# lambdaclass/simpleworks

Hardware: AMD Instinct MI355X
Metric: Marlin prove() constraints/sec at 2^20 R1CS; G1 MSM points/sec (higher is better)
Workload: dtype u32 limbs (384-bit Montgomery Fq for G1, 256-bit Fr); 1 GPU; marlin_prove: synthetic R1CS, 2^20 constraints = variables = non-zeros per matrix (|H| = |K| = 2^20), SRS + proving key device resident; per_gpu_units=1048576, multi_gpu=replicas (one proof per rank)

## Files before the change

### simpleworks_amd/_lib.py

```python
import ctypes
import json
import os

import numpy as np

_HERE = os.path.dirname(os.path.abspath(__file__))
LIB_PATH = os.environ.get("SWM_LIB_PATH") or os.path.join(_HERE, "libswmarlin.so")

_u64p = ctypes.POINTER(ctypes.c_uint64)
_u32p = ctypes.POINTER(ctypes.c_uint32)
_vp = ctypes.c_void_p
_sz = ctypes.c_size_t
_int = ctypes.c_int

ABI = {
    "swm_version": (_int, []),
    "swm_strerror": (ctypes.c_char_p, [_int]),
    "swm_init": (_int, [_int, ctypes.POINTER(_vp)]),
    "swm_destroy": (None, [_vp]),
    "swm_last_error": (ctypes.c_char_p, [_vp]),
    "swm_set_stream": (_int, [_vp, _vp]),
    "swm_set_msm_sharding": (_int, [_vp, ctypes.c_uint, ctypes.c_uint, _vp, _vp]),
    "swm_rccl_unique_id": (_int, [ctypes.c_void_p]),
    "swm_rccl_init": (_int, [_vp, ctypes.c_void_p, ctypes.c_uint, ctypes.c_uint]),
# ... 427 lines not shown
    def selftest_poly_eval(self, p_mont, z_mont):
        p = np.ascontiguousarray(p_mont, dtype=np.uint64).reshape(-1, 4)
        out = np.zeros(4, dtype=np.uint64)
        self._poly(2, p, p.shape[0], 0, z_mont, None, out)
        return out

    def selftest_poly_eval_many(self, buf_mont, pieces, z_mont):
        buf = np.ascontiguousarray(buf_mont, dtype=np.uint64).reshape(-1, 4)
        pc = np.asarray(pieces, dtype=np.uint64).reshape(-1, 2)
        out = np.zeros((pc.shape[0], 4), dtype=np.uint64)
        self._poly(3, buf, buf.shape[0], 0, z_mont, pc, out)
        return out

    def selftest_ntt_from(self, src_mont, log_n, inverse=False, coset=False):
        src = np.ascontiguousarray(src_mont, dtype=np.uint64).reshape(-1, 4).copy()
        out = np.zeros((1 << log_n, 4), dtype=np.uint64)
        self._poly(4 + int(bool(inverse)) + 2 * int(bool(coset)), src, src.shape[0], log_n, None, None, out)
        return out, src

    def selftest_ntt_cosets(self, coeffs_mont, log_n, ks):
        src = np.ascontiguousarray(coeffs_mont, dtype=np.uint64).reshape(-1, 4).copy()
        kk = np.ascontiguousarray(ks, dtype=np.uint64).reshape(-1)
        out = np.zeros((kk.size << log_n, 4), dtype=np.uint64)
        self._check(self.lib.swm_selftest_poly(self.h, 9, src.ctypes.data, src.shape[0], log_n, _p64(np.zeros(4, np.uint64)),
                                               _p64(kk), kk.size, out.ctypes.data), "swm_selftest_poly")
        return out.reshape(kk.size, 1 << log_n, 4)

    def selftest_intt_cosets3(self, evals_mont, log_n):
        ev = np.ascontiguousarray(evals_mont, dtype=np.uint64).reshape(-1, 4).copy()
        out = np.zeros_like(ev)
        self._poly(10, ev, ev.shape[0], log_n, None, None, out)
        return out

    def selftest_scan(self, words):
        w = np.ascontiguousarray(words, dtype=np.uint32).reshape(-1)
        out = np.zeros(w.size + 1, dtype=np.uint32)
        self._poly(8, w, w.size, 0, None, None, out)
        return out[:-1], int(out[-1])

    def selftest_sample_fr(self, rng, need):
        out = np.zeros((max(need, 1), 4), dtype=np.uint64)
        self._check(self.lib.swm_selftest_sample_fr(self.h, rng.h, need, _p64(out)), "swm_selftest_sample_fr")
        return out[:need]

    def selftest_mul_throughput(self, which, threads, iters):
        ms = ctypes.c_float(0)
        self._check(self.lib.swm_selftest_mul_throughput(self.h, which, threads, iters, ctypes.byref(ms)),
                    "swm_selftest_mul_throughput")
        return ms.value
```

### simpleworks_amd/csrc/devops.cuh

```cuda
#pragma once
#include <chrono>
#include <exception>
#include <functional>
#include <utility>
#include <atomic>
#include "context.h"
#include "ff.cuh"
#include "fill.cuh"
#include "fr29.cuh"
#include "host/chacha.h"
#include "host/marlin_types.h"

namespace swm {

int ntt_run(swm_ctx* ctx, void* d_data, unsigned log_n, int inverse, int coset);
int ntt_run_from(swm_ctx* ctx, void* d_data, unsigned log_n, int inverse, int coset, const void* first_src, size_t src_len);
int ntt_cosets_fwd(swm_ctx* ctx, const void* coeffs, size_t len, unsigned log_n, const unsigned* ks, unsigned ncos, void* out);
int ntt_cosets_inv(swm_ctx* ctx, void* data, unsigned log_n, unsigned ncos);
int ntt_sharded_run(swm_ctx* ctx, void* d_local, unsigned log_n, int inverse, int blocks_in);
struct SpmvPlanHost {
    uint64_t nnz = 0, max_row = 0;
    std::vector<uint32_t> chunks, lrows;
};
struct SpmvPlan {
    uint64_t nnz = 0, max_row = 0;
    const uint32_t* d_chunks = nullptr;
    const uint32_t* d_lrows = nullptr;
    uint32_t n_chunks = 0, n_lrows = 0;
};
void spmv_plan_build(const uint32_t* rowptr, size_t rows, SpmvPlanHost* plan);
int spmv_run(swm_ctx* ctx, const void* d_rowptr, const void* d_col, const void* d_val, const void* d_z, void* d_out,
             size_t rows, const SpmvPlan* plan = nullptr);
int batch_inverse_run(swm_ctx* ctx, void* d, size_t n);

inline void hip_check(swm_ctx* ctx, hipError_t e, const char* what) {
    if (e != hipSuccess) {
        set_err(ctx, SWM_ERR_HIP, "%s: %s", what, hipGetErrorString(e));
        throw MarlinError(e == hipErrorOutOfMemory ? SWM_ERR_OOM : SWM_ERR_HIP, std::string(what) + ": " + hipGetErrorString(e));
    }
}
inline void rc_check(swm_ctx* ctx, int rc) {
    if (rc != SWM_OK) throw MarlinError(rc, ctx->err);
}

template <class T>
struct DBuf {
    swm_ctx* ctx = nullptr;
    T* p = nullptr;
    size_t n = 0, cap = 0;
    DBuf() {}
    DBuf(swm_ctx* c, size_t count) : ctx(c), n(count) {
// ... 829 lines not shown
```

### simpleworks_amd/csrc/marlin.hip

```cpp
#include <stdlib.h>
#include <string.h>
#include <unistd.h>
#include <algorithm>
#include <chrono>
#include <functional>
#include <memory>
#include "devops.cuh"
#include "g1.cuh"
#include "host/ahp.h"

#include "msm.h"
using namespace swm;

#define LAUNCHX(ctx, name, kernel, grid, block, shmem, ...)                         \
    do {                                                                            \
        prof_begin(ctx, name);                                                      \
        hipLaunchKernelGGL(kernel, grid, block, shmem, (ctx)->stream, __VA_ARGS__); \
        prof_end(ctx);                                                              \
        hip_check(ctx, hipGetLastError(), name);                                    \
    } while (0)

#include "host/pk_codec.h"
#include "host/host_handles.h"
struct swm_srs {
// ... 1009 lines not shown
        poly[H] = fp_add(poly[H], rho);
    });
}
void div_vh(swm_ctx* ctx, const Fr* q, size_t part, size_t total, Fr* h, Fr* g) {
    ew(ctx, "div_vh", 3 * part, [=] __device__(size_t j) {
        Fr acc = q[j + part];
        if (j + 2 * part < total) acc = fp_add(acc, q[j + 2 * part]);
        if (j + 3 * part < total) acc = fp_add(acc, q[j + 3 * part]);
        h[j] = acc;
        if (j < part) g[j] = fp_add(q[j], acc);
    });
}
void div_vk(swm_ctx* ctx, const Fr* q, size_t part, size_t total, Fr* h) {
    ew(ctx, "div_vk", 3 * part, [=] __device__(size_t j) {
        Fr acc = fp_zero<Fr>();
        for (uint64_t i = 1; j + i * part < total; i++) acc = fp_add(acc, q[j + i * part]);
        h[j] = acc;
    });
}
#ifndef SWM_OUTER_COSETS
#define SWM_OUTER_COSETS 1
#endif
static constexpr uint64_t OUTER_COSETS_MIN_H = 16;
struct Cosets3 {
    Fr p0, p1, p2;
};
__device__ __forceinline__ Cosets3 cosets3_solve(const Fr& u0, const Fr& u1, const Fr& u2, const Fr& iota, const Fr& half) {
    const Fr p1 = fp_mul(fp_sub(u0, u2), half);
    const Fr e = fp_mul(fp_add(u0, u2), half);
    const Fr d = fp_sub(u1, fp_mul(iota, p1));
    return {fp_mul(fp_add(e, d), half), p1, fp_mul(fp_sub(e, d), half)};
}
static Fr fr_half() { return fp_inv(fp_from_u64<Fr>(2)); }
struct RAlphaNumerators {
    Fr n0, n1, n2, n3;
};
RAlphaNumerators r_alpha_numerators(const Fr& alpha, unsigned logH, uint64_t M) {
    Fr aH = alpha;
    for (unsigned i = 0; i < logH; i++) aH = fp_sqr(aH);
    Fr i4 = HDomain(M).gen;
    for (unsigned i = 0; i < logH; i++) i4 = fp_sqr(i4);
    return {fp_sub(aH, fp_one<Fr>()), fp_sub(aH, i4), fp_sub(aH, fp_sqr(i4)), fp_sub(aH, fp_mul(fp_sqr(i4), i4))};
}
struct IndexOnB {
    const Fr *ar, *ac, *arc, *av;
    const Fr *br, *bc, *brc, *bv;
    const Fr *cr, *cc, *crc, *cv;
};
struct Round3Challenges {
    Fr alpha, beta, ab, eta_a, eta_b, eta_c, vhab;
};
__device__ __forceinline__ Fr round3_a_minus_bf(const IndexOnB& x, const Round3Challenges& c, size_t i, const Fr& f) {
    Fr da = fp_add(fp_sub(fp_sub(c.ab, fp_mul(x.ar[i], c.alpha)), fp_mul(c.beta, x.ac[i])), x.arc[i]);
    Fr db = fp_add(fp_sub(fp_sub(c.ab, fp_mul(x.br[i], c.alpha)), fp_mul(c.beta, x.bc[i])), x.brc[i]);
    Fr dc = fp_add(fp_sub(fp_sub(c.ab, fp_mul(x.cr[i], c.alpha)), fp_mul(c.beta, x.cc[i])), x.crc[i]);
    Fr dbc = fp_mul(db, dc);
    Fr t = fp_add(fp_add(fp_mul(fp_mul(c.eta_a, x.av[i]), dbc), fp_mul(fp_mul(fp_mul(c.eta_b, x.bv[i]), da), dc)),
                  fp_mul(fp_mul(fp_mul(c.eta_c, x.cv[i]), da), db));
    Fr a_val = fp_mul(c.vhab, t);
    Fr b_val = fp_mul(da, dbc);
    return fp_sub(a_val, fp_mul(b_val, f));
}
struct ProveState {
    ChaChaRng& zk;
    PhaseTrace& tr;
    const ProveShape shape;
// ... 353 lines not shown
                q[k] = fp_sub(fp_mul(rh[k], summed), fp_mul(zk, th[k]));
            });
        }
        dv_ntt(ctx, s.t_poly, pk.logH, true);
    }
    s.tr.tick("r2: t polynomial enqueued");
    s.P_t.p = s.t_poly.p;
    s.P_t.n = H;
    pc_commit_begin(ctx, pk, &s.lane, s.P_t.p, s.P_t.n, false, 0, false, &s.j2[0]);
}

void round2_q1_cosets(swm_ctx* ctx, const swm_pk& pk, ProveState& s) {
    const uint64_t H = s.H;
    const Fr eta_a = s.st.eta_a, eta_b = s.st.eta_b, eta_c = s.st.eta_c;
    if (!s.ra_closed_form) {
        DVec ra_poly = dv_ntt_from(ctx, s.r_alpha_evals.p, H, pk.logH, true);
        DVec e12 = on_cosets12(ctx, s, ra_poly.p, H);
        s.e_ra = DVec(ctx, 3 * H);
        hip_check(ctx, hipMemcpyAsync(s.e_ra.p + H, e12.p, 2 * H * sizeof(Fr), hipMemcpyDeviceToDevice, ctx->stream), "copy");
    }
    {
        DVec e_t = on_cosets12(ctx, s, s.t_poly.p, H);
        Fr* out = s.q1.p + H;
        const Fr *pra = s.e_ra.p + H, *pza = s.e_za.p, *pzb = s.e_zb.p, *pt = e_t.p, *pz = s.e_z.p;
        ew(ctx, "round2_pointwise", 2 * H, [=] __device__(size_t i) {
            Fr a = pza[i], b = pzb[i];
            Fr summed = fp_add(fp_add(fp_mul(eta_c, fp_mul(a, b)), fp_mul(eta_a, a)), fp_mul(eta_b, b));
            out[i] = fp_sub(fp_mul(pra[i], summed), fp_mul(pz[i], pt[i]));
        });
        s.e_za.release();
        s.e_zb.release();
        s.e_z.release();
    }
    rc_check(ctx, ntt_cosets_inv(ctx, s.q1.p, pk.logH, 3));
    s.h1 = DVec(ctx, 3 * H);
    s.g1x = DVec(ctx, H);
    const Fr* q = s.q1.p;
    const Fr* mp = s.mask.p;
    Fr *h = s.h1.p, *g = s.g1x.p;
    const Fr iota = HDomain(4).gen, half = fr_half();
    ew(ctx, "q1_cosets_solve_div_vh", H, [=] __device__(size_t j) {
        const Cosets3 c = cosets3_solve(q[j], q[j + H], q[j + 2 * H], iota, half);
        const Fr p0 = fp_add(c.p0, mp[j]), p1 = fp_add(c.p1, mp[j + H]), p2 = fp_add(c.p2, mp[j + 2 * H]);
        const Fr hj = fp_add(p1, p2);
        h[j] = hj;
        h[j + H] = p2;
        h[j + 2 * H] = fp_zero<Fr>();
        g[j] = fp_add(p0, hj);
    });
}
void round2_q1(swm_ctx* ctx, const swm_pk& pk, ProveState& s) {
    if (s.cosets) return round2_q1_cosets(ctx, pk, s);
    const uint64_t H = s.H, M = s.M;
    const size_t Mloc = s.sp.Mloc;
    const Fr eta_a = s.st.eta_a, eta_b = s.st.eta_b, eta_c = s.st.eta_c;
    s.q1 = DVec(ctx, Mloc);
    {
        if (!s.ra_closed_form) {
            DVec ra_poly = dv_ntt_from(ctx, s.r_alpha_evals.p, H, pk.logH, true);
            s.e_ra = on_mul_domain(ctx, s, ra_poly.p, H);
        }
        DVec e_t = on_mul_domain(ctx, s, s.t_poly.p, H);
        Fr* out = s.q1.p;
        const Fr *pra = s.e_ra.p, *pza = s.e_za.p, *pzb = s.e_zb.p, *pt = e_t.p, *pz = s.e_z.p;
        ew(ctx, "round2_pointwise", Mloc, [=] __device__(size_t i) {
            Fr a = pza[i], b = pzb[i];
            Fr summed = fp_add(fp_add(fp_mul(eta_c, fp_mul(a, b)), fp_mul(eta_a, a)), fp_mul(eta_b, b));
// ... 30 lines not shown
    ew(ctx, "shard_interleave", 3 * H, [=] __device__(size_t i) {
        const size_t r = i & (((size_t)1 << lg) - 1), j = i >> lg;
        ph[i] = pa[r * 4 * Hl + j];
        if (i < Hl << lg) pg[i] = pa[r * 4 * Hl + 3 * Hl + j];
    });
}

void round2_commitments(swm_ctx* ctx, const swm_pk& pk, ProveState& s) {
    const uint64_t H = s.H;
    s.P_g1.p = s.g1x.p + 1; s.P_g1.n = H - 1; s.P_g1.has_bound = true; s.P_g1.bound = H - 2; s.P_g1.hiding = true;
    s.P_h1.p = s.h1.p; s.P_h1.n = 2 * H + 1;
    pc_commit_begin(ctx, pk, &s.lane, s.P_h1.p, s.P_h1.n, false, 0, false, &s.j2[2]);
    pc_commit_begin(ctx, pk, &s.lane, s.P_g1.p, s.P_g1.n, true, H - 2, true, &s.j2[1]);
    commit_flush(ctx);
    Fr rem0 = s.g1x.download(0, 1)[0];
    bool unsat = !fp_is_zero(rem0);
    pc_commit_blind(pk, &s.j2[0], nullptr, &s.P_t.rand);
    pc_commit_blind(pk, &s.j2[1], &s.zk, &s.P_g1.rand);
    pc_commit_blind(pk, &s.j2[2], nullptr, &s.P_h1.rand);
    commit_gather(ctx, {&s.j2[0].plain, &s.j2[1].plain, &s.j2[1].shifted, &s.j2[2].plain});
    pc_commit_end_round(ctx, pk, {&s.j2[0], &s.j2[1], &s.j2[2]}, {nullptr, &s.zk, nullptr},
                        {&s.P_t.rand, &s.P_g1.rand, &s.P_h1.rand}, s.comms2.data());
    if (unsat && !ctx->emulated_exchange)
        throw MarlinError(SWM_ERR_UNSATISFIED, "outer sumcheck does not hold: constraint system is not satisfied");
}

void round3_polys(swm_ctx* ctx, const swm_pk& pk, ProveState& s) {
    const uint64_t K = s.K, Bsz = s.Bsz;
    const Fr alpha = s.st.alpha, beta = s.st.beta;
    const Fr eta_a = s.st.eta_a, eta_b = s.st.eta_b, eta_c = s.st.eta_c;
    const Fr vhab = fp_mul(s.dh.vanishing(alpha), s.dh.vanishing(beta));
    s.f = DVec(ctx, K);
    const bool f_cosets = SWM_OUTER_COSETS && !s.sp.r3 && Bsz == 4 * K && K >= OUTER_COSETS_MIN_H;
    DVec f_K;
    {
        DVec inv(ctx, 3 * K);
        for (int m = 0; m < 3; m++) {
            Fr* out = inv.p + (size_t)m * K;
            const Fr *rk = pk.ar[m].row_K.p, *ck = pk.ar[m].col_K.p;
            ew(ctx, "round3_den_K", K, [=] __device__(size_t i) { out[i] = fp_mul(fp_sub(beta, rk[i]), fp_sub(alpha, ck[i])); });
        }
        rc_check(ctx, batch_inverse_run(ctx, inv.p, 3 * K));
        Fr* out = s.f.p;
        const Fr *ia = inv.p, *ib = inv.p + K, *ic = inv.p + 2 * K;
        const Fr *va = pk.ar[0].val_K.p, *vb = pk.ar[1].val_K.p, *vc = pk.ar[2].val_K.p;
        if (f_cosets) {
            f_K = DVec(ctx, K);
            out = f_K.p;
        }
        ew(ctx, "round3_f_K", K, [=] __device__(size_t i) {
            Fr t = fp_add(fp_add(fp_mul(fp_mul(eta_a, va[i]), ia[i]), fp_mul(fp_mul(eta_b, vb[i]), ib[i])),
                          fp_mul(fp_mul(eta_c, vc[i]), ic[i]));
            out[i] = fp_mul(vhab, t);
        });
        if (f_cosets) rc_check(ctx, ntt_run_from(ctx, s.f.p, pk.logK, 1, 0, f_K.p, K));
        else dv_ntt(ctx, s.f, pk.logK, true);
    }
    s.P_g2.p = s.f.p + 1; s.P_g2.n = K - 1; s.P_g2.has_bound = true; s.P_g2.bound = K - 2;
    pc_commit_begin(ctx, pk, &s.lane, s.P_g2.p, s.P_g2.n, true, K - 2, false, &s.j3[0]);
    s.h2 = DVec(ctx, 3 * K);
    const IndexOnB ix{pk.ar[0].row_B.p, pk.ar[0].col_B.p, pk.ar[0].row_col_B.p, pk.ar[0].val_B.p,
                      pk.ar[1].row_B.p, pk.ar[1].col_B.p, pk.ar[1].row_col_B.p, pk.ar[1].val_B.p,
                      pk.ar[2].row_B.p, pk.ar[2].col_B.p, pk.ar[2].row_col_B.p, pk.ar[2].val_B.p};
    const Round3Challenges ch{alpha, beta, fp_mul(beta, alpha), eta_a, eta_b, eta_c, vhab};
    if (s.sp.r3) {
        const size_t Bloc = Bsz / s.sp.SG, Bblk = Bloc / s.sp.SG, Kl = K / s.sp.SG, s_rank = s.sp.rank;
        DVec e_f = shard_evals(ctx, s.sp, s.f.p, K, pk.logB);
        DVec ab(ctx, Bloc);
        Fr* out = ab.p;
        const Fr* pf = e_f.p;
        ew(ctx, "round3_pointwise_B", Bloc, [=] __device__(size_t p) {
            const size_t i = Bloc * (p / Bblk) + s_rank * Bblk + (p % Bblk);
            out[p] = round3_a_minus_bf(ix, ch, i, pf[p]);
        });
        rc_check(ctx, ntt_sharded_run(ctx, ab.p, pk.logB, 1, 1));
        DVec loc(ctx, 3 * Kl);
        div_vk(ctx, ab.p, Kl, Bloc, loc.p);
        shard_gather_cyclic(ctx, loc.p, 3 * Kl, s.sp.slog_g, s.h2.p, 3 * K);
    } else if (f_cosets) {
        static const unsigned ks[3] = {1, 2, 3};
        DVec e_f(ctx, 3 * K);
        rc_check(ctx, ntt_cosets_fwd(ctx, s.f.p, K, pk.logK, ks, 3, e_f.p));
        DVec ab(ctx, Bsz);
        Fr* out = ab.p;
        const Fr *pf = e_f.p, *fk = f_K.p;
        const unsigned logK = pk.logK;
        ew(ctx, "round3_pointwise_B", Bsz, [=] __device__(size_t i) {
            const size_t k = i & 3, j = i >> 2;
            out[i] = round3_a_minus_bf(ix, ch, i, k ? pf[((k - 1) << logK) + j] : fk[j]);
        });
        dv_ntt(ctx, ab, pk.logB, true);
        div_vk(ctx, ab.p, K, Bsz, s.h2.p);
    } else {
        DVec e_f = dv_ntt_from(ctx, s.f.p, K, pk.logB, false);
        DVec ab(ctx, Bsz);
        Fr* out = ab.p;
        const Fr* pf = e_f.p;
        ew(ctx, "round3_pointwise_B", Bsz, [=] __device__(size_t i) { out[i] = round3_a_minus_bf(ix, ch, i, pf[i]); });
        dv_ntt(ctx, ab, pk.logB, true);
        div_vk(ctx, ab.p, K, Bsz, s.h2.p);
    }
    s.P_h2.p = s.h2.p;
    s.P_h2.n = 3 * K >= 3 ? 3 * K - 3 : 0;
}

std::vector<Fr> evaluations(swm_ctx* ctx, const swm_pk& pk, ProveState& s) {
    std::map<std::pair<std::string, bool>, Fr> eval_cache;
    {
        std::vector<std::pair<std::string, bool>> want;
        for (const char* l : {"z_b", "t", "g_1", "mask_poly", "z_a", "w", "h_1"}) want.push_back({l, false});
        for (int i = 0; i < 12; i++) want.push_back({kIndexerPolys[i], true});
// ... 710 lines not shown
    SWM_ON_DEVICE(ctx);
    SWM_GUARD(ctx, *out = pk_deserialize(ctx, bytes, len));
}
int swm_r1cs_is_satisfied(swm_ctx* ctx, const swm_r1cs* cs, int* ok, size_t* first_bad) {
    if (!ctx || !cs || !ok) return SWM_ERR_INVALID_ARG;
    SWM_ON_DEVICE(ctx);
    SWM_GUARD(ctx, is_satisfied_impl(ctx, cs, ok, first_bad));
}

static void selftest_poly_impl(swm_ctx* ctx, int op, void* data, size_t n, size_t m, const uint64_t* z, const uint64_t* pieces,
                               size_t npieces, void* out) {
    Fr zz = fp_zero<Fr>();
    if (z) memcpy(zz.v, z, 32);
    if (op == 8) {
        DBuf<uint32_t> in(ctx, n), res(ctx, n);
        if (n) in.upload((const uint32_t*)data, n);
        const uint32_t total = scan_exclusive_u32(ctx, in.p, res.p, n);
        std::vector<uint32_t> h = res.download(0, n);
        if (n) memcpy(out, h.data(), n * 4);
        ((uint32_t*)out)[n] = total;
        return;
    }
    DVec a(ctx, n);
    if (n) a.upload((const Fr*)data, n);
    if (op == 9) {
        unsigned ks[4];
        for (size_t c = 0; c < npieces; c++) ks[c] = (unsigned)pieces[c];
        DVec t(ctx, npieces << m);
        rc_check(ctx, ntt_cosets_fwd(ctx, a.p, n, (unsigned)m, ks, (unsigned)npieces, t.p));
        std::vector<Fr> h = t.download(0, t.n);
        memcpy(out, h.data(), t.n * sizeof(Fr));
        return;
    }
    if (op == 10) {
        const size_t N = (size_t)1 << m;
        rc_check(ctx, ntt_cosets_inv(ctx, a.p, (unsigned)m, 3));
        DVec t(ctx, 3 * N);
        const Fr* u = a.p;
        Fr* o = t.p;
        const Fr iota = HDomain(4).gen, half = fr_half();
        ew(ctx, "cosets3_solve", N, [=] __device__(size_t j) {
            const Cosets3 c = cosets3_solve(u[j], u[j + N], u[j + 2 * N], iota, half);
            o[j] = c.p0;
            o[j + N] = c.p1;
            o[j + 2 * N] = c.p2;
        });
        std::vector<Fr> h = t.download(0, t.n);
        memcpy(out, h.data(), t.n * sizeof(Fr));
        return;
    }
    if (op == 0) {
        suffix_recurrence(ctx, a.p, n, m, zz);
        std::vector<Fr> h = a.download(0, n);
        if (n) memcpy(data, h.data(), n * sizeof(Fr));
    } else if (op == 1) {
        DivResult r = div_linear(ctx, a.p, n, zz);
        std::vector<Fr> h = r.work.download(0, n);
        if (n) memcpy(out, h.data(), n * sizeof(Fr));
    } else if (op == 2) {
        const Fr v = poly_eval(ctx, a.p, n, zz);
        memcpy(out, v.v, sizeof(Fr));
    } else if (op == 3) {
        for (size_t i = 0; i < npieces; i++)
            if (pieces[2 * i] > n || pieces[2 * i + 1] > n - pieces[2 * i]) throw MarlinError(SWM_ERR_INVALID_ARG, "piece out of range");
        DVec res(ctx, npieces);
        std::vector<EvalItem> items;
        for (size_t i = 0; i < npieces; i++) items.push_back({a.p + pieces[2 * i], (size_t)pieces[2 * i + 1], res.p + i});
        EvalPoint ep = eval_point(ctx, zz);
        poly_eval_many(ctx, items, ep);
        std::vector<Fr> h = res.download(0, npieces);
        if (npieces) memcpy(out, h.data(), npieces * sizeof(Fr));
    } else {
        DVec t = dv_ntt_from(ctx, a.p, n, (unsigned)m, ((op - 4) & 1) != 0, ((op - 4) & 2) != 0);
        std::vector<Fr> h = t.download(0, t.n);
        memcpy(out, h.data(), t.n * sizeof(Fr));
        std::vector<Fr> s = a.download(0, n);
        if (n) memcpy(data, s.data(), n * sizeof(Fr));
    }
}
int swm_selftest_poly(swm_ctx* ctx, int op, void* data, size_t n, size_t m, const uint64_t z[4], const uint64_t* pieces,
                      size_t npieces, void* out) {
    if (!ctx || op < 0 || op > 10 || (n && !data)) return SWM_ERR_INVALID_ARG;
    if ((op >= 1 && op <= 3 && !z) || (op == 0 && (!z || m == 0)) || (op != 0 && !out) || (op == 3 && npieces && !pieces))
        return SWM_ERR_INVALID_ARG;
    if (op >= 4 && op <= 7 && (m < 1 || m > 28 || n > ((size_t)1 << m))) return SWM_ERR_INVALID_ARG;
    if (op == 9) {
        if (m < 1 || m > 26 || n > ((size_t)2 << m) || npieces < 1 || npieces > 4 || !pieces) return SWM_ERR_INVALID_ARG;
        for (size_t c = 0; c < npieces; c++)
            if (pieces[c] > 3) return SWM_ERR_INVALID_ARG;
    }
    if (op == 10 && (m < 1 || m > 26 || n != ((size_t)3 << m))) return SWM_ERR_INVALID_ARG;
    SWM_ON_DEVICE(ctx);
    SWM_GUARD(ctx, selftest_poly_impl(ctx, op, data, n, m, z, pieces, npieces, out));
}
static void selftest_sample_impl(swm_ctx* ctx, ChaChaRng& rng, size_t need, uint64_t* out_mont) {
    DVec d(ctx, need);
    sample_fr_bulk(ctx, rng, d.p, need);
    std::vector<Fr> h = d.download(0, need);
    if (need) memcpy(out_mont, h.data(), need * sizeof(Fr));
}
int swm_selftest_sample_fr(swm_ctx* ctx, swm_rng* rng, size_t need, uint64_t* out_mont) {
    if (!ctx || !rng || (need && !out_mont)) return SWM_ERR_INVALID_ARG;
    SWM_ON_DEVICE(ctx);
    SWM_GUARD(ctx, selftest_sample_impl(ctx, rng->r, need, out_mont));
}

}

extern "C" int swm_selftest_pairing(unsigned* failed) {
    using namespace swm;
    if (!failed) return SWM_ERR_INVALID_ARG;
    static const uint32_t gx[12] = SWM_G1_GEN_X_MONT, gy[12] = SWM_G1_GEN_Y_MONT;
    G1Affine P;
    for (int i = 0; i < 12; i++) {
        P.x.v[i] = gx[i];
        P.y.v[i] = gy[i];
    }
    G2Affine Q = g2_identity();
    for (unsigned s = 1; s < 200 && Q.inf; s++) {
        Fq2 x = {fp_from_u64<Fq>(s), fp_from_u64<Fq>(1)}, y;
        if (fq2_sqrt(x * x * x + g2_coeff_b(), &y)) {
            static const uint32_t cof[SWM_G2_COFACTOR_LIMBS] = SWM_G2_COFACTOR;
            Q = g2_mul({x, y, false}, cof, SWM_G2_COFACTOR_LIMBS);
        }
// ... 23 lines not shown
```

### simpleworks_amd/csrc/ntt.hip

```cpp
#include <atomic>
#include "context.h"
#include "ff.cuh"
#include "fr29.cuh"
#include <string.h>
#include <algorithm>
#include <vector>

namespace swm {

static constexpr int NTT_THREADS = 256;
static constexpr unsigned NTT_MAX_LOG_R = 10;

struct NttPassArgs {
    const Fr* src;
    Fr* dst;
    unsigned log_n, log_r, log_ns;
    const Fr* tw_small;
    const Fr* tw_lo;
    const Fr* tw_hi;
    const Fr* cs_lo;
    const Fr* cs_hi;
    uint64_t src_len;
    const Fr* pass_tw;
    int coset_in;
    int scale_out;
    int coset_out;
    Fr n_inv;
    uint64_t src_cstride, dst_cstride;
    uint32_t cos_k[4];
    int fold_in;
    Fr fold[4];
};

__device__ __forceinline__ Fr two_level_pow(const Fr* lo, const Fr* hi, uint64_t e) {
    Fr a = lo[e & 1023];
    uint64_t h = e >> 10;
    if (h) a = fp_mul(a, hi[h]);
    return a;
}

__device__ __forceinline__ unsigned bitrev_u(unsigned x, unsigned bits) { return bits ? (__brev(x) >> (32 - bits)) : 0u; }

template <int J>
__global__ void __launch_bounds__(NTT_THREADS) ntt_pass(NttPassArgs a) {
    SWM_LIGHT_KERNEL();
    extern __shared__ __align__(16) unsigned char smem_raw[];
    Fr* tile = reinterpret_cast<Fr*>(smem_raw);
    const unsigned R = 1u << a.log_r;
    const uint64_t n = 1ull << a.log_n;
    const uint64_t stride = n >> a.log_r;
    const uint64_t j0 = (uint64_t)blockIdx.x * J;
    const uint64_t ns_mask = (1ull << a.log_ns) - 1;
    const unsigned tw_shift = a.log_n - a.log_ns - a.log_r;
    const Fr* src = a.src + blockIdx.y * a.src_cstride;
    Fr* dst = a.dst + blockIdx.y * a.dst_cstride;
    const uint64_t cs_k = a.cos_k[blockIdx.y];
    for (unsigned e0 = 0; e0 < R * J; e0 += 4 * NTT_THREADS) {
        Fr xs[4];
#pragma unroll
        for (int u = 0; u < 4; u++) {
// ... 41 lines not shown
            unsigned p = qq & (hh - 1), blk = qq / hh;
            unsigned i0 = blk * 2 * h + p, i1 = i0 + hh, i2 = i0 + h, i3 = i2 + hh;
            Fr x0 = tile[i0 * J + jj], x1 = tile[i1 * J + jj], x2 = tile[i2 * J + jj], x3 = tile[i3 * J + jj];
            Fr a0 = fp_add(x0, x2), a2 = fp_sub(x0, x2);
            if (p) a2 = fp_mul(a2, a.tw_small[p * s1]);
            Fr a1 = fp_add(x1, x3), a3 = fp_mul(fp_sub(x1, x3), a.tw_small[(p + hh) * s1]);
            Fr y1 = fp_sub(a0, a1), y3 = fp_sub(a2, a3);
            if (p) {
                Fr w = a.tw_small[p * s2];
                y1 = fp_mul(y1, w);
                y3 = fp_mul(y3, w);
            }
            tile[i0 * J + jj] = fp_add(a0, a1);
            tile[i1 * J + jj] = y1;
            tile[i2 * J + jj] = fp_add(a2, a3);
            tile[i3 * J + jj] = y3;
        }
        __syncthreads();
    }
    for (unsigned e = threadIdx.x; e < R * J; e += NTT_THREADS) {
        unsigned jj, u;
        if (a.log_ns == 0) {
            u = e % R;
            jj = e / R;
        } else {
            jj = e % J;
            u = e / J;
        }
        uint64_t j = j0 + jj;
        uint64_t k = j & ns_mask;
        uint64_t o = ((j - k) << a.log_r) + k + ((uint64_t)u << a.log_ns);
        Fr x = tile[bitrev_u(u, a.log_r) * J + jj];
        if (a.scale_out) {
            Fr s = a.n_inv;
            if (a.coset_out) s = fp_mul(s, two_level_pow(a.cs_lo, a.cs_hi, o * cs_k));
            x = fp_mul(x, s);
        }
        dst[o] = x;
    }
}

struct LazyPlan {
    Spread29 r2;
    Spread29 s1[6];
    Spread29 s2[6];
    Spread29 s4;
    uint32_t reduce;
    uint32_t out_below_2r;
};
struct NttLazyArgs {
    NttPassArgs a;
    LazyPlan plan;
    int last_pass;
};
__device__ __forceinline__ Fr29 two_level_pow29(const Fr* lo, const Fr* hi, uint64_t e) {
    Fr29 a = fr29_unpack(lo[e & 1023]);
    uint64_t h = e >> 10;
    if (h) a = fr29_mul_fenced(a, fr29_unpack(hi[h]));
    return a;
}
__device__ __forceinline__ unsigned tile_slot(unsigned idx) { return (idx + (idx >> 5)) * 9; }
__device__ __forceinline__ void tile_put(uint32_t* tile, unsigned idx, const Fr29& x) {
    const unsigned o = tile_slot(idx);
#pragma unroll
    for (int i = 0; i < 9; i++) tile[o + i] = x.l[i];
}
__device__ __forceinline__ Fr29 tile_get(const uint32_t* tile, unsigned idx) {
// ... 75 lines not shown
                Fr29 x0 = tile_get(tile, i0 * J + jj), x2 = tile_get(tile, i2 * J + jj);
                a0 = fr29_add(x0, x2);
                a2 = fr29_mul_fenced(fr29_sub(x0, x2, S1), fr29_unpack(a.tw_small[p * s1]));
            }
            {
                Fr29 x1 = tile_get(tile, i1 * J + jj), x3 = tile_get(tile, i3 * J + jj);
                a1 = fr29_add(x1, x3);
                a3 = fr29_mul_fenced(fr29_sub(x1, x3, S1), fr29_unpack(a.tw_small[(p + hh) * s1]));
            }
            const Fr29 w = fr29_unpack(a.tw_small[p * s2]);
            Fr29 y0 = fr29_add(a0, a1);
            y0 = red ? fr29_mul_fenced(y0, fr29_const(Fr29Consts::ONE)) : fr29_normalize(y0);
            tile_put(tile, i0 * J + jj, y0);
            tile_put(tile, i1 * J + jj, fr29_mul_fenced(fr29_sub(a0, a1, S2), w));
            tile_put(tile, i2 * J + jj, fr29_normalize(fr29_add(a2, a3)));
            tile_put(tile, i3 * J + jj, fr29_mul_fenced(fr29_sub(a2, a3, P.s4), w));
        }
        __syncthreads();
    }
    for (unsigned e = threadIdx.x; e < R * J; e += NTT_THREADS) {
        unsigned jj, u;
        if (a.log_ns == 0) {
            u = e % R;
            jj = e / R;
        } else {
            jj = e % J;
            u = e / J;
        }
        uint64_t j = j0 + jj;
        uint64_t k = j & ns_mask;
        uint64_t o = ((j - k) << a.log_r) + k + ((uint64_t)u << a.log_ns);
        Fr29 x = tile_get(tile, bitrev_u(u, a.log_r) * J + jj);
        if (a.scale_out) {
            Fr29 sc = fr29_unpack(a.n_inv);
            if (a.coset_out) sc = fr29_mul_fenced(two_level_pow29(a.cs_lo, a.cs_hi, o * cs_k), sc);
            x = fr29_canonical(fr29_mul_fenced(x, sc), true);
        } else if (args.last_pass) {
            x = fr29_canonical(x, P.out_below_2r != 0);
        }
        dst[o] = fr29_pack(x);
    }
}

static Fr host_root_of_unity(unsigned log_n, bool inverse) {
    Fr w;
    const uint32_t root[8] = SWM_FR_ROOT47_MONT;
    for (int i = 0; i < 8; i++) w.v[i] = root[i];
    for (unsigned i = log_n; i < 47; i++) w = fp_sqr(w);
    if (inverse) w = fp_inv(w);
    return w;
}

static int upload_powers(swm_ctx* ctx, const Fr& base, size_t count, void** out, bool lazy29 = false) {
    std::vector<Fr> h(count);
    Fr cur = lazy29 ? fp_from_u64<Fr>(32) : fp_one<Fr>();
    for (size_t i = 0; i < count; i++) {
        h[i] = cur;
        cur = fp_mul(cur, base);
    }
    SWM_HIP(ctx, hipMalloc(out, count * sizeof(Fr)));
    SWM_HIP(ctx, hipMemcpy(*out, h.data(), count * sizeof(Fr), hipMemcpyHostToDevice));
    return SWM_OK;
}

static int two_level_tables(swm_ctx* ctx, const Fr& base, size_t max_exp, NttTables* t, bool lazy29 = false) {
    SWM_TRY(upload_powers(ctx, base, 1024, &t->lo, lazy29));
    Fr b1024 = base;
// ... 95 lines not shown
        uint64_t t = (uint64_t)Fr29Consts::P[i] * k + carry;
        sp.l[i] = i < 8 ? (uint32_t)(t & M29) : (uint32_t)t;
        carry = t >> 29;
    }
    sp.l[0] += borrows << 29;
    for (int i = 1; i < 8; i++) sp.l[i] += (borrows << 29) - borrows;
    sp.l[8] -= borrows;
    return sp;
}
static LazyPlan lazy_plan(unsigned log_r, unsigned b_in) {
    LazyPlan P;
    memset(&P, 0, sizeof(P));
    unsigned B = b_in;
    P.r2 = lazy_spread(2 * B, 1);
    if (log_r & 1) B = std::max(2 * B, 2u);
    const unsigned nsteps = log_r / 2;
    for (unsigned st = 0; st < nsteps && st < 6; st++) {
        P.s1[st] = lazy_spread(2 * B, 1);
        P.s2[st] = lazy_spread(4 * B, 2);
        const bool red = 4 * B > 64 || st + 1 == nsteps;
        if (red) P.reduce |= 1u << st;
        B = red ? 4 : 4 * B;
    }
    P.s4 = lazy_spread(4, 1);
    P.out_below_2r = B <= 2 ? 1u : 0u;
    return P;
}

int ntt_run_from(swm_ctx* ctx, void* d_data, unsigned log_n, int inverse, int coset, const void* first_src, size_t src_len);
int ntt_run(swm_ctx* ctx, void* d_data, unsigned log_n, int inverse, int coset) {
    return ntt_run_from(ctx, d_data, log_n, inverse, coset, nullptr, 0);
}
static int ntt_run_multi(swm_ctx* ctx, void* d_data, unsigned log_n, int inverse, int coset, const void* first_src, size_t src_len,
                         unsigned ncos, const unsigned* ks);
int ntt_run_from(swm_ctx* ctx, void* d_data, unsigned log_n, int inverse, int coset, const void* first_src, size_t src_len) {
    if (first_src && src_len > (1ull << std::min(log_n, 62u))) src_len = 1ull << log_n;
    return ntt_run_multi(ctx, d_data, log_n, inverse, coset ? 1 : 0, first_src, src_len, 1, nullptr);
}
int ntt_cosets_fwd(swm_ctx* ctx, const void* coeffs, size_t len, unsigned log_n, const unsigned* ks, unsigned ncos, void* out) {
    if (ncos < 1 || ncos > 4 || log_n > 28 || len > (2ull << log_n)) return set_err(ctx, SWM_ERR_INVALID_ARG, "ntt cosets: bad shape");
    for (unsigned c = 0; c < ncos; c++)
        if (ks[c] > 3) return set_err(ctx, SWM_ERR_INVALID_ARG, "ntt cosets: coset index > 3");
    return ntt_run_multi(ctx, out, log_n, 0, 2, coeffs, len, ncos, ks);
}
int ntt_cosets_inv(swm_ctx* ctx, void* data, unsigned log_n, unsigned ncos) {
    if (ncos < 1 || ncos > 4 || log_n > 28) return set_err(ctx, SWM_ERR_INVALID_ARG, "ntt cosets: bad shape");
    const unsigned ks[4] = {0, 1, 2, 3};
    return ntt_run_multi(ctx, data, log_n, 1, 2, nullptr, 0, ncos, ks);
}
static int ntt_run_multi(swm_ctx* ctx, void* d_data, unsigned log_n, int inverse, int coset, const void* first_src, size_t src_len,
                         unsigned ncos, const unsigned* ks) {
    if (log_n > 30) return set_err(ctx, SWM_ERR_INVALID_ARG, "ntt: log_n > 30 unsupported");
    const uint64_t n = 1ull << log_n;
    for (unsigned c = 0; c < ncos; c++) {
        ctx->stat_ntt_calls++;
        ctx->log_call('n', log_n);
        ctx->stat_ntt_elems += n;
    }
    Fr* data = reinterpret_cast<Fr*>(d_data);
    const uint64_t total = n * ncos;
    const unsigned maxr = NTT_MAX_LOG_R;
    static const bool lazy = env_switch("SWM_NTT_LAZY", 1, 0, 1) != 0;
    NttTables *rt = nullptr, *ct = nullptr;
    SWM_TRY(get_root_tables_form(ctx, log_n, inverse, lazy, &rt));
    if (coset == 1) SWM_TRY(get_coset_tables(ctx, log_n, inverse, &ct, lazy));
    if (coset == 2) SWM_TRY(get_root_tables_form(ctx, log_n + 2, inverse, lazy, &ct));
    Fr fold[4];
    for (unsigned c = 0; c < 4; c++) {
        fold[c] = fp_one<Fr>();
        if (coset == 2 && c < ncos)
            for (unsigned e = 0; e < ks[c]; e++) fold[c] = fp_mul(fold[c], host_root_of_unity(2, false));
    }
    Fr n_inv = fp_one<Fr>();
    if (inverse) n_inv = fp_inv(fp_from_u64<Fr>(n));
    if (lazy) n_inv = fp_mul(n_inv, fp_from_u64<Fr>(32));
    unsigned npass = log_n <= maxr ? 1 : (log_n + maxr - 1) / maxr;
    unsigned radices[8];
    {
        unsigned rem = log_n;
        for (unsigned p = 0; p < npass; p++) {
            unsigned r = (rem + (npass - p) - 1) / (npass - p);
            radices[p] = r;
            rem -= r;
        }
    }
    Fr *tmp = nullptr, *tmp2 = nullptr;
    SWM_TRY(scratch(ctx, "ntt.tmp", total * sizeof(Fr), (void**)&tmp));
    if (npass % 2 == 1 && npass >= 3) SWM_TRY(scratch(ctx, "ntt.tmp2", total * sizeof(Fr), (void**)&tmp2));
    const Fr* src = first_src ? reinterpret_cast<const Fr*>(first_src) : data;
    if (npass == 1 && !first_src) {
        SWM_HIP(ctx, hipMemcpyAsync(tmp, data, total * sizeof(Fr), hipMemcpyDeviceToDevice, ctx->stream));
        src = tmp;
    }
    unsigned log_ns = 0;
    for (unsigned p = 0; p < npass; p++) {
        NttPassArgs a;
        a.src = src;
        if (p == npass - 1) a.dst = data;
        else if (tmp2) a.dst = (p % 2 == 0) ? tmp : tmp2;
        else a.dst = (src == tmp) ? data : tmp;
        a.src_len = (p == 0 && first_src) ? (uint64_t)src_len : n;
        a.log_n = log_n;
        a.log_r = radices[p];
        a.log_ns = log_ns;
        SWM_TRY(get_small_table(ctx, a.log_r, inverse, &a.tw_small, lazy));
        a.tw_lo = reinterpret_cast<const Fr*>(rt->lo);
        a.tw_hi = reinterpret_cast<const Fr*>(rt->hi);
        a.cs_lo = ct ? reinterpret_cast<const Fr*>(ct->lo) : nullptr;
        a.cs_hi = ct ? reinterpret_cast<const Fr*>(ct->hi) : nullptr;
        a.pass_tw = nullptr;
        if (lazy && log_ns != 0) SWM_TRY(get_pass_table(ctx, log_n, inverse, log_ns, a.log_r, rt, &a.pass_tw));
        a.coset_in = (coset && !inverse && p == 0) ? 1 : 0;
        a.scale_out = (inverse && p == npass - 1) ? 1 : 0;
        a.coset_out = (coset && inverse && p == npass - 1) ? 1 : 0;
        a.n_inv = n_inv;
        a.src_cstride = (p == 0 && first_src) ? 0 : n;
        a.dst_cstride = n;
        a.fold_in = (coset == 2 && a.coset_in && src_len > n) ? 1 : 0;
        for (unsigned c = 0; c < 4; c++) {
            a.cos_k[c] = coset == 2 ? (c < ncos ? ks[c] : 0) : 1;
            a.fold[c] = fold[c];
        }
        uint64_t cols = n >> a.log_r;
        if (lazy) {
            NttLazyArgs la;
            la.a = a;
            la.plan = lazy_plan(a.log_r, (p > 0 || a.coset_in) ? 2u : 1u);
            la.last_pass = p == npass - 1 ? 1 : 0;
            unsigned J = 1;
            if (npass > 1) {
                J = (log_n >= 19 ? 1024u : 512u) >> a.log_r;
                if (J < 1) J = 1;
                if (J > 16) J = 16;
                while (J > cols) J >>= 1;
            }
            const size_t elems = (size_t)J << a.log_r;
            size_t shmem = (elems + (elems >> 5) + 1) * 36;
            if (shmem < 64) shmem = 64;
            dim3 grid((unsigned)(cols / J), ncos), block(NTT_THREADS);
            if (shmem > 64 * 1024) {
                static std::atomic<size_t> granted[64];
                if (J != 1 || shmem > 160 * 1024) return set_err(ctx, SWM_ERR_INVALID_ARG, "ntt: tile does not fit LDS");
                if (granted[ctx->device & 63].load() < shmem) {
                    SWM_HIP(ctx, hipFuncSetAttribute((const void*)ntt_pass_lazy<1>, hipFuncAttributeMaxDynamicSharedMemorySize, (int)shmem));
                    granted[ctx->device & 63].store(shmem);
                }
            }
            switch (J) {
                case 1: SWM_LAUNCH(ctx, "ntt_pass", ntt_pass_lazy<1>, grid, block, shmem, la); break;
                case 2: SWM_LAUNCH(ctx, "ntt_pass", ntt_pass_lazy<2>, grid, block, shmem, la); break;
                case 4: SWM_LAUNCH(ctx, "ntt_pass", ntt_pass_lazy<4>, grid, block, shmem, la); break;
                case 8: SWM_LAUNCH(ctx, "ntt_pass", ntt_pass_lazy<8>, grid, block, shmem, la); break;
                default: SWM_LAUNCH(ctx, "ntt_pass", ntt_pass_lazy<16>, grid, block, shmem, la); break;
            }
// ... 98 lines not shown
```

Before: 22.64 million constraints/s.

## Compute round-3 h2 via coset inverse NTTs with fused vanishing-inverse scaling

Adds a round-3 path for h2. It evaluates f on cosets 1..3, forms a-bf pointwise, and inverse-NTTs each coset with a per-coset output scale that folds in 1/v_K on that coset. A 3x3 solve then recombines the cosets into h2's three coefficient pieces. This replaces the previous division-by-vanishing handling on the f_cosets path, which is meant to drop separate division or scaling passes. The NTT kernel argument n_inv becomes a per-coset out_scale array indexed by blockIdx.y, and f_K is released early to save memory.

```diff
diff --git a/simpleworks_amd/_lib.py b/simpleworks_amd/_lib.py
--- a/simpleworks_amd/_lib.py
+++ b/simpleworks_amd/_lib.py
@@ -483,6 +483,19 @@
         self._poly(10, ev, ev.shape[0], log_n, None, None, out)
         return out
 
+    def selftest_intt_cosets(self, evals_mont, log_n, ks, scales_mont=None):
+        ev = np.ascontiguousarray(evals_mont, dtype=np.uint64).reshape(-1, 4).copy()
+        kk = np.ascontiguousarray(ks, dtype=np.uint64).reshape(-1)
+        flag = np.zeros(4, dtype=np.uint64)
+        pc = kk
+        if scales_mont is not None:
+            flag[0] = 1
+            pc = np.concatenate([kk, np.ascontiguousarray(scales_mont, dtype=np.uint64).reshape(kk.size * 4)])
+        out = np.zeros_like(ev)
+        self._check(self.lib.swm_selftest_poly(self.h, 11, ev.ctypes.data, ev.shape[0], log_n, _p64(flag), _p64(pc), kk.size,
+                                               out.ctypes.data), "swm_selftest_poly")
+        return out.reshape(kk.size, 1 << log_n, 4)
+
     def selftest_scan(self, words):
         w = np.ascontiguousarray(words, dtype=np.uint32).reshape(-1)
         out = np.zeros(w.size + 1, dtype=np.uint32)
diff --git a/simpleworks_amd/csrc/devops.cuh b/simpleworks_amd/csrc/devops.cuh
--- a/simpleworks_amd/csrc/devops.cuh
+++ b/simpleworks_amd/csrc/devops.cuh
@@ -16,7 +16,7 @@
 int ntt_run(swm_ctx* ctx, void* d_data, unsigned log_n, int inverse, int coset);
 int ntt_run_from(swm_ctx* ctx, void* d_data, unsigned log_n, int inverse, int coset, const void* first_src, size_t src_len);
 int ntt_cosets_fwd(swm_ctx* ctx, const void* coeffs, size_t len, unsigned log_n, const unsigned* ks, unsigned ncos, void* out);
-int ntt_cosets_inv(swm_ctx* ctx, void* data, unsigned log_n, unsigned ncos);
+int ntt_cosets_inv(swm_ctx* ctx, void* data, unsigned log_n, const unsigned* ks, unsigned ncos, const void* scale = nullptr);
 int ntt_sharded_run(swm_ctx* ctx, void* d_local, unsigned log_n, int inverse, int blocks_in);
 struct SpmvPlanHost {
     uint64_t nnz = 0, max_row = 0;
diff --git a/simpleworks_amd/csrc/marlin.hip b/simpleworks_amd/csrc/marlin.hip
--- a/simpleworks_amd/csrc/marlin.hip
+++ b/simpleworks_amd/csrc/marlin.hip
@@ -1065,6 +1065,23 @@
     return {fp_mul(fp_add(e, d), half), p1, fp_mul(fp_sub(e, d), half)};
 }
 static Fr fr_half() { return fp_inv(fp_from_u64<Fr>(2)); }
+#ifndef SWM_H2_COSETS
+#define SWM_H2_COSETS 1
+#endif
+__device__ __forceinline__ Cosets3 cosets123_solve(const Fr& u1, const Fr& u2, const Fr& u3, const Fr& half_iota_inv, const Fr& half) {
+    const Fr p1 = fp_mul(fp_sub(u1, u3), half_iota_inv);
+    const Fr d = fp_mul(fp_add(u1, u3), half);
+    const Fr e = fp_add(u2, p1);
+    return {fp_mul(fp_add(e, d), half), p1, fp_mul(fp_sub(e, d), half)};
+}
+static void vk_inv_on_cosets123(Fr out[3]) {
+    const Fr i4 = HDomain(4).gen;
+    Fr p = fp_one<Fr>();
+    for (int k = 0; k < 3; k++) {
+        p = fp_mul(p, i4);
+        out[k] = fp_inv(fp_sub(p, fp_one<Fr>()));
+    }
+}
 struct RAlphaNumerators {
     Fr n0, n1, n2, n3;
 };
@@ -1484,7 +1501,8 @@
         s.e_zb.release();
         s.e_z.release();
     }
-    rc_check(ctx, ntt_cosets_inv(ctx, s.q1.p, pk.logH, 3));
+    static const unsigned ks012[3] = {0, 1, 2};
+    rc_check(ctx, ntt_cosets_inv(ctx, s.q1.p, pk.logH, ks012, 3));
     s.h1 = DVec(ctx, 3 * H);
     s.g1x = DVec(ctx, H);
     const Fr* q = s.q1.p;
@@ -1581,6 +1599,7 @@
     const Fr vhab = fp_mul(s.dh.vanishing(alpha), s.dh.vanishing(beta));
     s.f = DVec(ctx, K);
     const bool f_cosets = SWM_OUTER_COSETS && !s.sp.r3 && Bsz == 4 * K && K >= OUTER_COSETS_MIN_H;
+    const bool h2_cosets = SWM_H2_COSETS && f_cosets;
     DVec f_K;
     {
         DVec inv(ctx, 3 * K);
@@ -1604,6 +1623,7 @@
         });
         if (f_cosets) rc_check(ctx, ntt_run_from(ctx, s.f.p, pk.logK, 1, 0, f_K.p, K));
         else dv_ntt(ctx, s.f, pk.logK, true);
+        if (h2_cosets) f_K.release();
     }
     s.P_g2.p = s.f.p + 1; s.P_g2.n = K - 1; s.P_g2.has_bound = true; s.P_g2.bound = K - 2;
     pc_commit_begin(ctx, pk, &s.lane, s.P_g2.p, s.P_g2.n, true, K - 2, false, &s.j3[0]);
@@ -1626,6 +1646,30 @@
         DVec loc(ctx, 3 * Kl);
         div_vk(ctx, ab.p, Kl, Bloc, loc.p);
         shard_gather_cyclic(ctx, loc.p, 3 * Kl, s.sp.slog_g, s.h2.p, 3 * K);
+    } else if (h2_cosets) {
+        static const unsigned ks[3] = {1, 2, 3};
+        DVec e_f(ctx, 3 * K);
+        rc_check(ctx, ntt_cosets_fwd(ctx, s.f.p, K, pk.logK, ks, 3, e_f.p));
+        DVec ab(ctx, 3 * K);
+        Fr* out = ab.p;
+        const Fr* pf = e_f.p;
+        const unsigned logK = pk.logK;
+        ew(ctx, "round3_pointwise_B", 3 * K, [=] __device__(size_t p) {
+            const size_t j = p / 3, c = p - 3 * j, at = (c << logK) + j;
+            out[at] = round3_a_minus_bf(ix, ch, 4 * j + c + 1, pf[at]);
+        });
+        Fr vk_inv[3];
+        vk_inv_on_cosets123(vk_inv);
+        rc_check(ctx, ntt_cosets_inv(ctx, ab.p, pk.logK, ks, 3, vk_inv));
+        const Fr* u = ab.p;
+        Fr* h = s.h2.p;
+        const Fr half = fr_half(), half_iota_inv = fp_mul(half, fp_inv(HDomain(4).gen));
+        ew(ctx, "h2_cosets_solve", K, [=] __device__(size_t j) {
+            const Cosets3 c = cosets123_solve(u[j], u[j + K], u[j + 2 * K], half_iota_inv, half);
+            h[j] = c.p0;
+            h[j + K] = c.p1;
+            h[j + 2 * K] = c.p2;
+        });
     } else if (f_cosets) {
         static const unsigned ks[3] = {1, 2, 3};
         DVec e_f(ctx, 3 * K);
@@ -2402,9 +2446,21 @@
         memcpy(out, h.data(), t.n * sizeof(Fr));
         return;
     }
+    if (op == 11) {
+        unsigned ks[4];
+        Fr scale[4];
+        for (size_t c = 0; c < npieces; c++) ks[c] = (unsigned)pieces[c];
+        const bool scaled = z && z[0] != 0;
+        if (scaled) memcpy(scale, pieces + npieces, npieces * sizeof(Fr));
+        rc_check(ctx, ntt_cosets_inv(ctx, a.p, (unsigned)m, ks, (unsigned)npieces, scaled ? scale : nullptr));
+        std::vector<Fr> h = a.download(0, n);
+        memcpy(out, h.data(), n * sizeof(Fr));
+        return;
+    }
     if (op == 10) {
         const size_t N = (size_t)1 << m;
-        rc_check(ctx, ntt_cosets_inv(ctx, a.p, (unsigned)m, 3));
+        static const unsigned ks012[3] = {0, 1, 2};
+        rc_check(ctx, ntt_cosets_inv(ctx, a.p, (unsigned)m, ks012, 3));
         DVec t(ctx, 3 * N);
         const Fr* u = a.p;
         Fr* o = t.p;
@@ -2450,7 +2506,7 @@
 }
 int swm_selftest_poly(swm_ctx* ctx, int op, void* data, size_t n, size_t m, const uint64_t z[4], const uint64_t* pieces,
                       size_t npieces, void* out) {
-    if (!ctx || op < 0 || op > 10 || (n && !data)) return SWM_ERR_INVALID_ARG;
+    if (!ctx || op < 0 || op > 11 || (n && !data)) return SWM_ERR_INVALID_ARG;
     if ((op >= 1 && op <= 3 && !z) || (op == 0 && (!z || m == 0)) || (op != 0 && !out) || (op == 3 && npieces && !pieces))
         return SWM_ERR_INVALID_ARG;
     if (op >= 4 && op <= 7 && (m < 1 || m > 28 || n > ((size_t)1 << m))) return SWM_ERR_INVALID_ARG;
@@ -2460,6 +2516,11 @@
             if (pieces[c] > 3) return SWM_ERR_INVALID_ARG;
     }
     if (op == 10 && (m < 1 || m > 26 || n != ((size_t)3 << m))) return SWM_ERR_INVALID_ARG;
+    if (op == 11) {
+        if (m < 1 || m > 26 || npieces < 1 || npieces > 4 || !pieces || n != (npieces << m)) return SWM_ERR_INVALID_ARG;
+        for (size_t c = 0; c < npieces; c++)
+            if (pieces[c] > 3) return SWM_ERR_INVALID_ARG;
+    }
     SWM_ON_DEVICE(ctx);
     SWM_GUARD(ctx, selftest_poly_impl(ctx, op, data, n, m, z, pieces, npieces, out));
 }
diff --git a/simpleworks_amd/csrc/ntt.hip b/simpleworks_amd/csrc/ntt.hip
--- a/simpleworks_amd/csrc/ntt.hip
+++ b/simpleworks_amd/csrc/ntt.hip
@@ -25,7 +25,7 @@
     int coset_in;
     int scale_out;
     int coset_out;
-    Fr n_inv;
+    Fr out_scale[4];
     uint64_t src_cstride, dst_cstride;
     uint32_t cos_k[4];
     int fold_in;
@@ -133,7 +133,7 @@
         uint64_t o = ((j - k) << a.log_r) + k + ((uint64_t)u << a.log_ns);
         Fr x = tile[bitrev_u(u, a.log_r) * J + jj];
         if (a.scale_out) {
-            Fr s = a.n_inv;
+            Fr s = a.out_scale[blockIdx.y];
             if (a.coset_out) s = fp_mul(s, two_level_pow(a.cs_lo, a.cs_hi, o * cs_k));
             x = fp_mul(x, s);
         }
@@ -275,7 +275,7 @@
         uint64_t o = ((j - k) << a.log_r) + k + ((uint64_t)u << a.log_ns);
         Fr29 x = tile_get(tile, bitrev_u(u, a.log_r) * J + jj);
         if (a.scale_out) {
-            Fr29 sc = fr29_unpack(a.n_inv);
+            Fr29 sc = fr29_unpack(a.out_scale[blockIdx.y]);
             if (a.coset_out) sc = fr29_mul_fenced(two_level_pow29(a.cs_lo, a.cs_hi, o * cs_k), sc);
             x = fr29_canonical(fr29_mul_fenced(x, sc), true);
         } else if (args.last_pass) {
@@ -437,7 +437,7 @@
     return ntt_run_from(ctx, d_data, log_n, inverse, coset, nullptr, 0);
 }
 static int ntt_run_multi(swm_ctx* ctx, void* d_data, unsigned log_n, int inverse, int coset, const void* first_src, size_t src_len,
-                         unsigned ncos, const unsigned* ks);
+                         unsigned ncos, const unsigned* ks, const Fr* scale = nullptr);
 int ntt_run_from(swm_ctx* ctx, void* d_data, unsigned log_n, int inverse, int coset, const void* first_src, size_t src_len) {
     if (first_src && src_len > (1ull << std::min(log_n, 62u))) src_len = 1ull << log_n;
     return ntt_run_multi(ctx, d_data, log_n, inverse, coset ? 1 : 0, first_src, src_len, 1, nullptr);
@@ -448,13 +448,14 @@
         if (ks[c] > 3) return set_err(ctx, SWM_ERR_INVALID_ARG, "ntt cosets: coset index > 3");
     return ntt_run_multi(ctx, out, log_n, 0, 2, coeffs, len, ncos, ks);
 }
-int ntt_cosets_inv(swm_ctx* ctx, void* data, unsigned log_n, unsigned ncos) {
+int ntt_cosets_inv(swm_ctx* ctx, void* data, unsigned log_n, const unsigned* ks, unsigned ncos, const void* scale) {
     if (ncos < 1 || ncos > 4 || log_n > 28) return set_err(ctx, SWM_ERR_INVALID_ARG, "ntt cosets: bad shape");
-    const unsigned ks[4] = {0, 1, 2, 3};
-    return ntt_run_multi(ctx, data, log_n, 1, 2, nullptr, 0, ncos, ks);
+    for (unsigned c = 0; c < ncos; c++)
+        if (ks[c] > 3) return set_err(ctx, SWM_ERR_INVALID_ARG, "ntt cosets: coset index > 3");
+    return ntt_run_multi(ctx, data, log_n, 1, 2, nullptr, 0, ncos, ks, reinterpret_cast<const Fr*>(scale));
 }
 static int ntt_run_multi(swm_ctx* ctx, void* d_data, unsigned log_n, int inverse, int coset, const void* first_src, size_t src_len,
-                         unsigned ncos, const unsigned* ks) {
+                         unsigned ncos, const unsigned* ks, const Fr* scale) {
     if (log_n > 30) return set_err(ctx, SWM_ERR_INVALID_ARG, "ntt: log_n > 30 unsupported");
     const uint64_t n = 1ull << log_n;
     for (unsigned c = 0; c < ncos; c++) {
@@ -518,13 +519,13 @@
         a.coset_in = (coset && !inverse && p == 0) ? 1 : 0;
         a.scale_out = (inverse && p == npass - 1) ? 1 : 0;
         a.coset_out = (coset && inverse && p == npass - 1) ? 1 : 0;
-        a.n_inv = n_inv;
         a.src_cstride = (p == 0 && first_src) ? 0 : n;
         a.dst_cstride = n;
         a.fold_in = (coset == 2 && a.coset_in && src_len > n) ? 1 : 0;
         for (unsigned c = 0; c < 4; c++) {
             a.cos_k[c] = coset == 2 ? (c < ncos ? ks[c] : 0) : 1;
             a.fold[c] = fold[c];
+            a.out_scale[c] = (scale && inverse && c < ncos) ? fp_mul(n_inv, scale[c]) : n_inv;
         }
         uint64_t cols = n >> a.log_r;
         if (lazy) {
```

New measurement: 22.48 million constraints/s. About the same (-0.7%).
